# slothfulxtx/Texture-GS

Hardware: AMD Instinct MI355X
Metric: fwd+bwd views/sec @800x800, 300k Gaussians + 1024^2 texture; HBM GB/s vs roofline (higher is better)
Workload: dtype f32; 1 GPU; c3: N=300000 Gaussians, cubemap 6x1024x1024x3 f32, 800x800, fwd+bwd, sh_degree 3; parallelism=views sharded dp1, view_pipeline=3 HIP streams, order=accumulate, forwards begun one view per stream ahead, grad_allreduce=none (1 GPU)

## Files before the change

### texture-gs_amd/build.py

```python
import os
import subprocess
import sys

HERE = os.path.dirname(os.path.abspath(__file__))
ROOT = os.path.dirname(HERE)
CSRC = os.path.join(HERE, "csrc")
OBJ = os.path.join(HERE, "build")
LIB = os.path.join(HERE, os.environ.get("TEXGS_LIB_NAME", "libtexgs.so"))
OBJ = os.path.join(HERE, os.environ.get("TEXGS_OBJ_DIR", "build"))
HIPCC = os.environ.get("HIPCC", "/opt/rocm/bin/hipcc")

COMMON = ["--offload-arch=gfx950", "-O3", "-std=c++17", "-fPIC", "-I" + os.path.join(ROOT, "include"),
          "-I" + CSRC, "-Wall"]
UNITS = {
    "preprocess.hip": ["-ffp-contract=off"],
    "binning.hip": [],
    "render.hip": ["-munsafe-fp-atomics", "-ffp-contract=fast", "-fno-slp-vectorize"],
    "loss.hip": [],
    "selftest.hip": [],
    "uvnet.hip": [],
    "uvmap.hip": ["-munsafe-fp-atomics"],
    "points.hip": ["-ffp-contract=off"],
    "cubetex.hip": ["-munsafe-fp-atomics"],
    "density.hip": ["-ffp-contract=off"],
    "abi.hip": [],
}
HEADERS = [os.path.join(CSRC, "common.h"), os.path.join(CSRC, "wave_ops.h"), os.path.join(CSRC, "render_bwd_body.h"),
           os.path.join(ROOT, "include", "texgs.h")]


def build_id():
    import hashlib
    h = hashlib.sha256()
    files = sorted(os.path.join(CSRC, f) for f in os.listdir(CSRC) if f.endswith((".hip", ".h"))) + [os.path.join(ROOT, "include", "texgs.h")]
    for f in files:
        h.update(os.path.basename(f).encode())
        h.update(open(f, "rb").read())
    h.update(repr((COMMON[:4], sorted(UNITS.items()), os.environ.get("TEXGS_EXTRA_FLAGS", ""))).encode())
    return h.hexdigest()[:16]


def _newer(src_list, target):
    if not os.path.exists(target):
        return True
    t = os.path.getmtime(target)
    return any(os.path.getmtime(s) > t for s in src_list)


def build(force=False, verbose=False):
    os.makedirs(OBJ, exist_ok=True)
    objs = []
    bid = build_id()
    idfile = os.path.join(OBJ, "build_id.txt")
    stale_id = not os.path.exists(idfile) or open(idfile).read().strip() != bid
    for src, flags in UNITS.items():
        sp = os.path.join(CSRC, src)
        op = os.path.join(OBJ, src.replace(".hip", ".o"))
        objs.append(op)
        if src == "abi.hip":
            flags = flags + ['-DTEXGS_BUILD_ID="%s"' % bid]
# ... 18 lines not shown
```

### texture-gs_amd/csrc/abi.hip

```cpp
#include "common.h"
#include <stdio.h>
#include <string.h>
#include <stdlib.h>

#include <mutex>
#include <vector>

namespace {

thread_local char g_err[512] = "";

struct EvRec { int kid; hipEvent_t a, b; };
std::mutex g_prof_mu;
bool g_prof_on = false;
uint32_t g_prof_mask = 0xFFFFFFFFu;
std::vector<EvRec> g_prof_log;
std::vector<hipEvent_t> g_prof_free;

hipEvent_t prof_event() {
    if (!g_prof_free.empty()) { hipEvent_t e = g_prof_free.back(); g_prof_free.pop_back(); return e; }
    hipEvent_t e; (void)hipEventCreate(&e); return e;
}

struct ProfScope {
// ... 98 lines not shown
    const size_t nw = texgs_num_rendered_words(num_gaussians);
    if (host_words < nw) return fail_msg("host buffer too small (texgs_num_rendered_words)");
    hipStream_t s = (hipStream_t)stream;
    hipError_t e = hipMemcpyAsync(host_pinned, bin_block_sums_ptr(geom, num_gaussians), nw * sizeof(uint32_t), hipMemcpyDeviceToHost, s);
    if (e != hipSuccess) return fail("num_rendered readback", e);
    if (sort_first) {
        TexGSFrame f0; memset(&f0, 0, sizeof(f0)); f0.num_gaussians = num_gaussians;
        if (int r = depth_sort_scan(&f0, const_cast<TexGSGeom*>(geom), s)) return r;
    }
    return 0;
}
int texgs_num_rendered_reduce(const uint32_t* host_pinned, int32_t num_gaussians, uint32_t* host_out, uint64_t* fingerprint_out) {
    if (!host_pinned || !host_out) return fail_msg("NULL argument");
    *host_out = 0;
    if (fingerprint_out) *fingerprint_out = 0;
    if (num_gaussians <= 0) return 0;
    const size_t nblk = ((size_t)num_gaussians + TG_BLOCK - 1) / TG_BLOCK;
    unsigned long long total = 0ull;
    uint32_t fa = 0u, fb = 0u;
    for (size_t k = 0; k < nblk; ++k) { total += host_pinned[k]; fa += host_pinned[nblk + k]; fb += host_pinned[2 * nblk + k]; }
    if (total > 0xFFFFFFFFull) return fail_msg("num_rendered exceeds 2^32 - 1 instances");
    *host_out = (uint32_t)total;
    if (fingerprint_out) *fingerprint_out = ((uint64_t)fb << 32) | (uint64_t)fa;
    return 0;
}

int texgs_depth_sort_scan(TexGSGeom* geom, int32_t num_gaussians, void* stream) {
    if (!geom) return fail_msg("NULL argument");
    TexGSFrame f0; memset(&f0, 0, sizeof(f0)); f0.num_gaussians = num_gaussians;
    return depth_sort_scan(&f0, geom, (hipStream_t)stream);
}

static int render_forward_impl(const TexGSFrame* frame, const TexGSInputs* in, const TexGSGeom* geom,
                               const TexGSBinning* bin, TexGSImage* img, void* stream, bool counters_zeroed) {
    if (int r = validate_frame(frame)) return r;
    if (!in || !geom || !bin || !img) return fail_msg("NULL argument");
    hipStream_t s = (hipStream_t)stream;
    const CamConst c = make_cam(frame);
    if (img->tex_bin_count && in->texture && !counters_zeroed) {
        hipError_t e = hipMemsetAsync(img->tex_bin_count, 0, sizeof(uint32_t) * 2 * tex_bin_count(c.R), s);
        if (e != hipSuccess) return fail("tex_bin_count memset", e);
    }
    { ProfScope p(TEXGS_K_RENDER_FWD, s); launch_render_fwd(c, frame, in, geom, bin, img, s); }
    return check(frame, s, "render_fwd");
}

int texgs_render_forward(const TexGSFrame* frame, const TexGSInputs* in, const TexGSGeom* geom,
                         const TexGSBinning* bin, TexGSImage* img, void* stream) {
    return render_forward_impl(frame, in, geom, bin, img, stream, false);
}

int texgs_bin_sort_render_forward(const TexGSFrame* frame, const TexGSInputs* in, const TexGSGeom* geom,
                                  TexGSBinning* bin, TexGSImage* img, void* stream) {
    if (int r = validate_frame(frame)) return r;
    if (!in || !geom || !bin || !img) return fail_msg("NULL argument");
    hipStream_t s = (hipStream_t)stream;
    const CamConst c = make_cam(frame);
    if (bin->num_rendered > 0) {
        if (bin->sort_temp_bytes < sort_temp_bytes(bin->num_rendered, (uint32_t)(c.tiles_x * c.tiles_y))) return fail_msg("sort_temp too small");
        { ProfScope p(TEXGS_K_DUPLICATE, s); launch_duplicate(c, geom, bin, s); }
        if (int r = check(frame, s, "duplicate_with_keys")) return r;
        { ProfScope p(TEXGS_K_SORT, s);
          if (int r = launch_sort(c, geom, bin, s)) return fail("tile sort", (hipError_t)r); }
        if (int r = check(frame, s, "tile sort")) return r;
    }
    { ProfScope p(TEXGS_K_RANGES, s);
      launch_ranges(c, bin, img->tex_bin_count, img->tex_bin_count ? 2 * (int)tex_bin_count(c.R) : 0, s); }
    if (int r = check(frame, s, "tile_ranges")) return r;
    return render_forward_impl(frame, in, geom, bin, img, stream, true);
}

int texgs_backward_render(const TexGSFrame* frame, const TexGSInputs* in, const TexGSGeom* geom,
                          const TexGSBinning* bin, const TexGSImage* img, TexGSGrads* grads, void* stream) {
    if (int r = validate_frame(frame)) return r;
    if (!in || !geom || !bin || !img || !grads) return fail_msg("NULL argument");
    if (!(grads->want & TEXGS_WANT_ALL)) return fail_msg("TexGSGrads.want is empty: ask for TEXGS_WANT_TEXTURE and / or TEXGS_WANT_GAUSSIANS");
    if ((grads->want & TEXGS_WANT_GAUSSIANS) && !grads->acc) return fail_msg("acc must be allocated (zero-filled) when Gaussian gradients are wanted");
    if ((grads->want & TEXGS_WANT_TEXTURE) && in->texture && !grads->dL_dtexture) return fail_msg("dL_dtexture must be allocated (zero-filled) when the texture gradient is wanted");
    if (!img->survivors || !img->surv_qmask || !img->surv_count)
        return fail_msg("the forward of this call left no survivor lists (TexGSImage.survivors / surv_qmask / surv_count were NULL): "
                        "run the forward with them to be able to run its backward");
    hipStream_t s = (hipStream_t)stream;
    const CamConst c = make_cam(frame);
    if (bin->num_rendered > 0) {
        { ProfScope p(TEXGS_K_RENDER_BWD, s); launch_render_bwd(c, frame, in, geom, bin, img, grads, s); }
        if (int r = check(frame, s, "render_bwd")) return r;
        if (tex_bins_enabled(c, in, img, grads)) {
            { ProfScope p(TEXGS_K_TEXGRAD_REDUCE, s); launch_texgrad_reduce(c, img, grads, s); }
            if (int r = check(frame, s, "texgrad_reduce")) return r;
        }
    }
    return 0;
}

int texgs_backward_preprocess(const TexGSFrame* frame, const TexGSInputs* in, const TexGSGeom* geom, TexGSGrads* grads,
                              void* stream) {
    if (int r = validate_frame(frame)) return r;
    if (!in || !geom || !grads) return fail_msg("NULL argument");
    if (!(grads->want & TEXGS_WANT_GAUSSIANS)) return 0;
    if (!grads->acc) return fail_msg("acc must be allocated");
    if (in->cov3D_precomp && !grads->dL_dcov3D) return fail_msg("dL_dcov3D is required with cov3D_precomp");
    hipStream_t s = (hipStream_t)stream;
// ... 321 lines not shown
```

### texture-gs_amd/csrc/common.h

```cpp
#pragma once
#include <hip/hip_runtime.h>
#include <stdint.h>
#include "texgs.h"

#define TG_NEAR_Z        0.2f
#define TG_LOWPASS       0.3f
#define TG_FRUSTUM_CLAMP 1.3f
#define TG_ALPHA_MAX     0.99f
#define TG_ALPHA_MIN     (1.0f / 255.0f)
#define TG_T_EPS         1e-4f
#define TG_PLANE_EPS     5e-2f
#define TG_DEN_MIN       0.2f
#define TG_MA_MIN        1e-20f
#define TG_SH_C0         0.28209479177387814f

enum {
    R_XY = 0, R_CONIC = 2, R_OP = 5, R_G2 = 6, R_GM = 8, R_PHI = 14, R_VD = 17, R_DEPTH = 20, R_N = 21
};
enum {
    M_P = 0, M_DEN = 6, M_DN = 9, M_PHI = 18, M_VD = 21, M_DEPTH = 24, M_N = 25
};

#define TG_BLOCK 256

struct CamConst {
    int W, H, tiles_x, tiles_y;
    float fx, fy, tanfovx, tanfovy;
    float scale_modifier;
    int sh_degree, sh_coeffs, R, N;
};

static inline CamConst make_cam(const TexGSFrame* f) {
    CamConst c;
    c.W = f->image_width; c.H = f->image_height;
    c.tiles_x = (c.W + TEXGS_TILE - 1) / TEXGS_TILE;
    c.tiles_y = (c.H + TEXGS_TILE - 1) / TEXGS_TILE;
    c.tanfovx = f->tanfovx; c.tanfovy = f->tanfovy;
    c.fx = (float)c.W / (2.0f * f->tanfovx);
    c.fy = (float)c.H / (2.0f * f->tanfovy);
    c.scale_modifier = f->scale_modifier;
    c.sh_degree = f->sh_degree; c.sh_coeffs = f->sh_coeffs; c.R = f->tex_res; c.N = f->num_gaussians;
    return c;
}

void launch_preprocess_fwd(const CamConst& c, const TexGSFrame* f, const TexGSInputs* in, TexGSGeom* g, hipStream_t s);
void launch_preprocess_bwd(const CamConst& c, const TexGSFrame* f, const TexGSInputs* in, const TexGSGeom* g,
                           TexGSGrads* gr, hipStream_t s);
void launch_mark_visible(const TexGSFrame* f, const float* means3D, uint8_t* visible, hipStream_t s);
int  launch_depth_sort_scan(const TexGSGeom* g, int N, hipStream_t s);
uint32_t* bin_block_sums_ptr(const TexGSGeom* g, int N);
uint32_t* bin_header_ptr(const TexGSGeom* g, int N, int* words);
size_t scan_temp_bytes(int N);
size_t sort_temp_bytes(uint32_t D, uint32_t T);
void launch_duplicate(const CamConst& c, const TexGSGeom* g, TexGSBinning* b, hipStream_t s);
int  launch_sort(const CamConst& c, const TexGSGeom* g, TexGSBinning* b, hipStream_t s);
void launch_ranges(const CamConst& c, TexGSBinning* b, uint32_t* zero_words, int num_zero_words, hipStream_t s);
void launch_render_fwd(const CamConst& c, const TexGSFrame* f, const TexGSInputs* in, const TexGSGeom* g,
                       const TexGSBinning* b, TexGSImage* img, hipStream_t s);
size_t tex_bin_count(int R);
bool tex_bins_enabled(const CamConst& c, const TexGSInputs* in, const TexGSImage* img, const TexGSGrads* gr);
void launch_texgrad_reduce(const CamConst& c, const TexGSImage* img, TexGSGrads* gr, hipStream_t s);
void launch_render_bwd(const CamConst& c, const TexGSFrame* f, const TexGSInputs* in, const TexGSGeom* g,
                       const TexGSBinning* b, const TexGSImage* img, TexGSGrads* gr, hipStream_t s);
int launch_rgb_alpha_loss(const float* image, const float* gt_image, const float* alpha, const float* gt_alpha, int H,
                          int W, float lambda_dssim, float lambda_alpha, float* scratch, float* sums, float* d_image,
                          float* d_alpha, hipStream_t s);
void launch_selftest_waveops(const float* seed128, float* out576, hipStream_t s);
int launch_geom_losses(const float* norm, const float* gt_norm, const float* gt_image, const float* mask, const float* depth,
                       const float* gt_depth, int H, int W, float lambda_norm, float lambda_smooth, float gamma,
                       float lambda_depth, float* sums, float* d_norm, float* d_depth, hipStream_t s);
int launch_norm_from_depth(const float* depth, const float* viewmatrix, float tanfovx, float tanfovy, int H, int W, float threshold,
                           float* out_norm, float* out_mask, hipStream_t s);
size_t uv_packed_bytes(int precision);
int launch_uv_pack(const TexGSUVNet* net, int precision, void* packed, hipStream_t s);
int launch_uv_taylor_packed(const TexGSUVNet* net, int precision, const void* packed, const float* xyz, int N, float* uvs, float* grad_uvs,
                            hipStream_t s);
size_t uv_backward_temp_bytes(int N);
int launch_uv_backward(const TexGSUVNet* net, const float* xyz, const float* g, int N, const TexGSUVNetGrad* out, void* temp, int mixed,
                       hipStream_t s);
int hashgrid_levels(const TexGSHashGrid* g, float* scale, uint32_t* res, uint32_t* size, uint32_t* offset, uint32_t* n_params);
int launch_hashgrid_forward(const TexGSHashGrid* g, const float* params, const float* x, int N, float* enc, hipStream_t s);
size_t hashgrid_backward_temp_bytes(const TexGSHashGrid* g, int N);
int launch_hashgrid_backward(const TexGSHashGrid* g, const float* params, const float* x, const float* d_enc, int N, float* d_params,
                             float* d_x, void* temp, hipStream_t s);
size_t chamfer_nn_temp_bytes(int P);
int launch_chamfer_nn(const float* a, int P, const float* b, int Q, float* d2, int32_t* idx, void* temp, hipStream_t s);
size_t sort_pairs32_temp_bytes(uint32_t n);
int launch_sort_pairs32(const uint32_t* keys_in, uint32_t n, int key_bits, uint32_t* keys_out, uint32_t* vals_out, void* temp, hipStream_t s);
size_t knn3_temp_bytes(int n);
int launch_knn3_mean_dist2(const float* xyz, int n, float* mean_d2, void* temp, hipStream_t s);
// ... 12 lines not shown
```

### texture-gs_amd/csrc/render.hip

```cpp
#include "common.h"
#include "wave_ops.h"

namespace {

typedef unsigned long long ull;

struct __attribute__((packed, aligned(4))) Texel3 { float x, y, z; };
__device__ __forceinline__ Texel3 load_texel(const float* __restrict__ tex, uint32_t boff) {
    return *reinterpret_cast<const Texel3*>(reinterpret_cast<const char*>(tex) + boff);
}

typedef uint32_t tg_u4 __attribute__((ext_vector_type(4)));
template <class T> __device__ __forceinline__ T nt_load(const T* p) {
    return __builtin_nontemporal_load(p);
}
template <class T> __device__ __forceinline__ void nt_store(T* p, T v) {
    __builtin_nontemporal_store(v, p);
}
__device__ __forceinline__ uint2 nt_load2(const uint2* p) {
    const unsigned long long v = nt_load(reinterpret_cast<const unsigned long long*>(p));
    return make_uint2((uint32_t)v, (uint32_t)(v >> 32));
}
__device__ __forceinline__ void nt_store2(uint2* p, uint2 v) {
    nt_store(reinterpret_cast<unsigned long long*>(p), (unsigned long long)v.x | ((unsigned long long)v.y << 32));
}

struct CubeTap {
    uint32_t o00, dox, doy;
    int   x0, y0;
    float fx, fy;
    float sc, tc, h, rma, sm, su, sv;
    int   axis, face;
};

// ... 105 lines not shown
#define KEY_OX(K)  ((int)(((K) >> 14) & 7u))
#define KEY_OY(K)  ((int)(((K) >> 17) & 7u))

__device__ __forceinline__ void lane_pixel(int lane, int& ox, int& oy) {
    ox = (((lane >> 4) & 1) << 2) | (lane & 3);
    oy = (((lane >> 5) & 1) << 2) | ((lane >> 2) & 3);
}

__device__ __forceinline__ void load_chunk(const PixArgs& a, Planes& P, int lane, bool live, uint32_t id, uint32_t pos,
                                           float4& T0, float4& T1) {
    const float4 z = make_float4(0.f, 0.f, 0.f, 0.f);
    float4 S0 = z, S1 = z, S2 = z, S3 = z, S4 = z;
    T0 = z; T1 = make_float4(0.f, 0.f, -1.f, 1.f);
    if (live) {
        const float4* __restrict__ tp = a.rec_test + 2 * (size_t)id;
        const float4* __restrict__ sp = a.rec_shade + (TEXGS_REC_SHADE_FLOATS / 4) * (size_t)id;
        T0 = tp[0]; T1 = tp[1]; S0 = sp[0]; S1 = sp[1]; S2 = sp[2]; S3 = sp[3]; S4 = sp[4];
    }
    P.A[lane] = T0;
    { float* pb = reinterpret_cast<float*>(&P.B[lane]); pb[0] = T1.x; pb[1] = T1.y; pb[2] = __uint_as_float(pos); }
    P.C[lane] = make_float4(S3.z, S3.w, S4.x, S4.y);
    P.D[lane] = S0; P.E[lane] = S1; P.F[lane] = S2;
    P.G[lane] = make_float2(S3.x, S3.y);
}
__device__ __forceinline__ void init_dummy(Planes& P, int lane) {
    if (lane == 0) {
        const float4 z = make_float4(0.f, 0.f, 0.f, 0.f);
        P.A[TG_DUMMY] = z; P.B[TG_DUMMY] = make_float4(0.f, 0.f, __uint_as_float(0xFFFFFFFFu), 0.f); P.C[TG_DUMMY] = z;
        P.D[TG_DUMMY] = z; P.E[TG_DUMMY] = z; P.F[TG_DUMMY] = z; P.G[TG_DUMMY] = make_float2(0.f, 0.f);
    }
}

#define FQ_CAP 128
struct __attribute__((aligned(16))) FwdLds {
    Planes p;
    uint2 q[FQ_CAP];
    ull col[64 * 3];
    uint32_t ring[TG_RING];
    uint8_t list[4][64];
    uint32_t ccnt[TG_RESV / 2];
};

template <bool TAPS>
__global__ void __launch_bounds__(64, 4)
k_render_fwd(PixArgs a, float* __restrict__ out_color, float* __restrict__ out_depth, float* __restrict__ out_norm,
             float* __restrict__ out_alpha, float* __restrict__ final_T, uint32_t* __restrict__ n_contrib,
             uint32_t* __restrict__ bin_count) {
    __shared__ FwdLds L;
    const int lane = (int)threadIdx.x;
    int tile, wave;
    if (!wave_block(a, tile, wave)) return;
    const int tile_x = tile % a.tiles_x, tile_y = tile / a.tiles_x;
    const int wave_px = tile_x * TEXGS_TILE + ((wave & 1) << 3), wave_py = tile_y * TEXGS_TILE + ((wave >> 1) << 3);
    int ox, oy;
    lane_pixel(lane, ox, oy);
    const int px = wave_px + ox, py = wave_py + oy;
    const bool inside = (px < a.W) && (py < a.H);
    const float pxf = (float)px, pyf = (float)py;
    const float wpx = (float)wave_px, wpy = (float)wave_py;
    const uint2 range = a.ranges[tile];
    const int todo = (int)(range.y - range.x);
    const float* __restrict__ tex = a.texture;
    const uint32_t keybase = ((uint32_t)lane << 8) | ((uint32_t)ox << 14) | ((uint32_t)oy << 17);
    const uint8_t* mylist = L.list[lane >> 4];
    const int nbins_row = (a.R + 31) >> 5;

    L.col[lane * 3 + 0] = 0ull; L.col[lane * 3 + 1] = 0ull; L.col[lane * 3 + 2] = 0ull;
    resv_bin(L.p, lane) = TG_RESV_EMPTY;
    if (lane < TG_RESV / 2) L.ccnt[lane] = 0u;
    init_dummy(L.p, lane);
    __builtin_amdgcn_wave_barrier();

    bool done = !inside;
    ull done_mask = TG_BALLOT(!inside);
    float T = 1.0f;
    float Dp = 0.f, N0 = 0.f, N1 = 0.f, N2 = 0.f, Al = 0.f;
    uint32_t last = 0;
    int qhead = 0, qtail = 0;

    int pn = 0;
    int p_pl = 0;
    float p_w = 0.f, p_fx = 0.f, p_fy = 0.f, p_vd0 = 0.f, p_vd1 = 0.f, p_vd2 = 0.f;
    Texel3 p00 = {0.f, 0.f, 0.f}, p01 = p00, p10 = p00, p11 = p00;
    auto finish = [&]() {
        if (lane < pn) {
            float t0 = 0.f, t1 = 0.f, t2 = 0.f;
            if constexpr (TAPS) {
                const float w00 = (1.f - p_fx) * (1.f - p_fy), w01 = p_fx * (1.f - p_fy);
                const float w10 = (1.f - p_fx) * p_fy,         w11 = p_fx * p_fy;
                t0 = w00 * p00.x + w01 * p01.x + w10 * p10.x + w11 * p11.x;
                t1 = w00 * p00.y + w01 * p01.y + w10 * p10.y + w11 * p11.y;
                t2 = w00 * p00.z + w01 * p01.z + w10 * p10.z + w11 * p11.z;
            }
            ull* cp = L.col + p_pl * 3;
            atomicAdd(cp + 0, (ull)(fminf(p_w * fmaxf(0.f, TG_SH_C0 * t0 + p_vd0 + 0.5f), 2.0e9f) * 4294967296.0f));
            atomicAdd(cp + 1, (ull)(fminf(p_w * fmaxf(0.f, TG_SH_C0 * t1 + p_vd1 + 0.5f), 2.0e9f) * 4294967296.0f));
            atomicAdd(cp + 2, (ull)(fminf(p_w * fmaxf(0.f, TG_SH_C0 * t2 + p_vd2 + 0.5f), 2.0e9f) * 4294967296.0f));
        }
        pn = 0;
    };
    auto drain = [&](int n_) {
        finish();
        uint2 e_ = make_uint2(0u, 0u);
        if (lane < n_) e_ = L.q[(qhead + lane) & (FQ_CAP - 1)];
        const int jj_ = KEY_J(e_.y);
        const float4 f_ = L.p.F[jj_];
        const float2 g2 = L.p.G[jj_];
        const float4 a4_ = L.p.A[jj_];
        const float2 b2_ = *reinterpret_cast<const float2*>(&L.p.B[jj_]);
        const float ipx_ = (float)(wave_px + KEY_OX(e_.y)), ipy_ = (float)(wave_py + KEY_OY(e_.y));
        const float araw_ = gauss_alpha_raw(b2_.y, gauss_power(a4_.z, a4_.w, b2_.x, a4_.x - ipx_, a4_.y - ipy_));
        const float T_ = __uint_as_float(e_.x);
        const float w_ = fminf(TG_ALPHA_MAX, araw_) * T_;
        if constexpr (TAPS) {
            const float2 xy = make_float2(a4_.x, a4_.y);
            const float4 d_ = L.p.D[jj_], e4 = L.p.E[jj_];
            const float dpx = ipx_ - xy.x, dpy = ipy_ - xy.y;
            const float den = 1.0f + d_.x * dpx + d_.y * dpy;
            const float inv = (den >= TG_DEN_MIN) ? __builtin_amdgcn_rcpf(den) : 0.0f;
            const float u0 = f_.x + (d_.z * dpx + d_.w * dpy) * inv;
            const float u1 = f_.y + (e4.x * dpx + e4.y * dpy) * inv;
            const float u2 = f_.z + (e4.z * dpx + e4.w * dpy) * inv;
            const CubeTap ct = cube_address(u0, u1, u2, a.R);
            p00 = load_texel(tex, ct.o00); p01 = load_texel(tex, ct.o00 + ct.dox);
            p10 = load_texel(tex, ct.o00 + ct.doy); p11 = load_texel(tex, ct.o00 + ct.doy + ct.dox);
            p_fx = ct.fx; p_fy = ct.fy;
            if (bin_count != nullptr) {
                const bool binned = (lane < n_) && tap_binned(ct);
                const uint32_t bin = tap_bin(ct, nbins_row);
                const int home = tap_home(ct);
                const bool hit = binned && resv_bin(L.p, home) == bin;
                if (hit) atomicAdd(&L.ccnt[home >> 1], 1u << ((home & 1) << 4));
                ull pend = TG_BALLOT(binned) & ~TG_BALLOT(hit);
                while (pend != 0ull) {
                    const int l0 = __ffsll((long long)pend) - 1;
                    const uint32_t b0 = (uint32_t)__builtin_amdgcn_readlane((int)bin, l0);
                    const int h0 = __builtin_amdgcn_readlane(home, l0);
                    const ull m = pend & TG_BALLOT(bin == b0);
                    const uint32_t e0 = resv_bin(L.p, h0);
                    if (lane == l0) {
                        const uint32_t n = (uint32_t)__popcll(m);
                        if (e0 == TG_RESV_EMPTY) { resv_bin(L.p, h0) = b0; atomicAdd(&L.ccnt[h0 >> 1], n << ((h0 & 1) << 4)); }
                        else atomicAdd(bin_count + 6 * nbins_row * nbins_row + b0, n);
                    }
                    __builtin_amdgcn_wave_barrier();
                    pend &= ~m;
                }
            }
        }
        p_w = w_; p_pl = KEY_PL(e_.y); p_vd0 = f_.w; p_vd1 = g2.x; p_vd2 = g2.y;
        pn = n_;
    };

    const size_t sbase = 4 * (size_t)range.x + (size_t)wave * (size_t)todo;
    int nsurv = 0;
    int r = 0, nq = 0, qh = 0;
    const float4 zt0 = make_float4(0.f, 0.f, 0.f, 0.f), zt1 = make_float4(0.f, 0.f, -1.f, 1.f);
    float4 nt0 = zt0, nt1 = zt1;
    if (lane < todo) {
        const float4* __restrict__ tp = a.rec_test + 2 * (size_t)a.point_list[range.x + lane];
        nt0 = tp[0]; nt1 = tp[1];
    }
    uint32_t nid = (64 + lane < todo) ? a.point_list[range.x + 64 + lane] : 0u;
    bool all_done = (~done_mask == 0ull);
    while (!all_done) {
        while (nq < 64 && r < todo) {
            const int idx = r + lane;
            const float4 t0 = nt0, t1 = nt1;
            r += 64;
            nt0 = zt0; nt1 = zt1;
            if (r + lane < todo) {
                const float4* __restrict__ tp = a.rec_test + 2 * (size_t)nid;
                nt0 = tp[0]; nt1 = tp[1];
            }
            nid = (r + 64 + lane < todo) ? a.point_list[range.x + r + 64 + lane] : 0u;
            const bool reach = block_reachable(t0.x, t0.y, t0.z, t0.w, t1.x, t1.w, t1.z, wpx, wpy, 7.0f);
            const ull m = TG_BALLOT(reach);
            if (reach) L.ring[(qh + nq + mbcnt64(m)) & (TG_RING - 1)] = (uint32_t)idx;
            nq += __popcll(m);
        }
        if (nq == 0) break;
        const int take = min(64, nq);
        __builtin_amdgcn_wave_barrier();
        uint32_t pos = 0xFFFFFFFFu, id = 0u;
        if (lane < take) {
            pos = L.ring[(qh + lane) & (TG_RING - 1)];
            id = a.point_list[range.x + pos];
        }
        qh = (qh + take) & (TG_RING - 1); nq -= take;
        float4 T0, T1;
        load_chunk(a, L.p, lane, lane < take, id, pos, T0, T1);
        reinterpret_cast<uint32_t*>(&L.list[0][0])[lane] = 0x40404040u;
        __builtin_amdgcn_wave_barrier();
        int len[4];
        uint32_t qbits = 0u;
#pragma unroll
        for (int q = 0; q < 4; ++q) {
            const bool rowdone = ((done_mask >> (16 * q)) & 0xFFFFull) == 0xFFFFull;
            const bool geo = (lane < take) &&
                block_reachable(T0.x, T0.y, T0.z, T0.w, T1.x, T1.w, T1.z, wpx + (float)((q & 1) << 2), wpy + (float)((q >> 1) << 2), 3.0f);
            qbits |= geo ? (1u << q) : 0u;
            const bool rq = geo && !rowdone;
            const ull m = TG_BALLOT(rq);
            len[q] = __popcll(m);
            if (rq) L.list[q][mbcnt64(m)] = (uint8_t)lane;
        }
        if (a.surv != nullptr) {
            if (lane < take) { nt_store2(a.surv + sbase + nsurv + lane, make_uint2(id, pos)); nt_store(a.surv_qm + sbase + nsurv + lane, (uint16_t)qbits); }
            nsurv += take;
        }
        __builtin_amdgcn_wave_barrier();
        int tmax = max(max(len[0], len[1]), max(len[2], len[3]));
        auto test_one = [&](const float4& A, const float4& B, const float4& Cc, const int j) -> bool {
                const float power = gauss_power(A.z, A.w, B.x, A.x - pxf, A.y - pyf);
                const float alpha = fminf(TG_ALPHA_MAX, gauss_alpha_raw(B.y, power));
                const ull m_ok = TG_BALLOT(power <= 0.0f) & ~done_mask & TG_BALLOT(alpha >= TG_ALPHA_MIN);
                if (m_ok == 0ull) return false;
                bool ok = (!done) && (power <= 0.0f) && (alpha >= TG_ALPHA_MIN);
                const float Tn = T * (1.0f - alpha);
                const ull m_kill = m_ok & TG_BALLOT(Tn < TG_T_EPS);
                if (ok && Tn < TG_T_EPS) { done = true; ok = false; }
                done_mask |= m_kill;
                const ull bal = m_ok & ~m_kill;
                if (bal != 0ull) {
                    if (ok) {
                        const float w = alpha * T;
                        Dp += w * Cc.x; N0 += w * Cc.y; N1 += w * Cc.z; N2 += w * Cc.w; Al += w;
                        L.q[(qtail + mbcnt64(bal)) & (FQ_CAP - 1)] = make_uint2(__float_as_uint(T), keybase | (uint32_t)j);
                        T = Tn;
                        last = __float_as_uint(B.z) + 1u;
                    }
                    qtail += __popcll(bal);
                    if (qtail - qhead >= 64) {
                        __builtin_amdgcn_wave_barrier();
                        drain(64);
                        qhead += 64;
                    }
                }
                if (m_kill != 0ull) {
                    if (~done_mask == 0ull) { all_done = true; return true; }
// ... 5 lines not shown
                }
            return false;
        };
        int jx = mylist[0], jy = mylist[1];
        float4 xA = L.p.A[jx], xB = L.p.B[jx], xC = L.p.C[jx];
        float4 yA = xA, yB = xB, yC = xC;
        for (int t = 0; t < tmax; t += 2) {
            yA = L.p.A[jy]; yB = L.p.B[jy]; yC = L.p.C[jy];
            const int j0 = jx;
            jx = mylist[min(t + 2, 63)];
            if (test_one(xA, xB, xC, j0)) break;
            if (t + 1 >= tmax) break;
            xA = L.p.A[jx]; xB = L.p.B[jx]; xC = L.p.C[jx];
            const int j1 = jy;
            jy = mylist[min(t + 3, 63)];
            if (test_one(yA, yB, yC, j1)) break;
        }
        if (qtail - qhead > 0) {
            __builtin_amdgcn_wave_barrier();
            drain(qtail - qhead);
            qhead = qtail;
        }
        __builtin_amdgcn_wave_barrier();
    }
    finish();
    __builtin_amdgcn_wave_barrier();
    if (TAPS && bin_count != nullptr) {
        const uint32_t b = resv_bin(L.p, lane), n = (L.ccnt[lane >> 1] >> ((lane & 1) << 4)) & 0xFFFFu;
        uint32_t off = 0u;
        if (b != TG_RESV_EMPTY) off = atomicAdd(bin_count + b, n);
        uint32_t* __restrict__ rv = a.resv + (size_t)(4 * tile + wave) * (3 * TG_RESV);
        nt_store(rv + lane, b); nt_store(rv + TG_RESV + lane, off); nt_store(rv + 2 * TG_RESV + lane, n);
    }
    if (a.surv_cnt != nullptr && lane == 0) a.surv_cnt[4 * tile + wave] = (uint32_t)nsurv;
    if (inside) {
        const int HW = a.W * a.H, pix = py * a.W + px;
        const double q = 1.0 / 4294967296.0;
        nt_store(out_color + pix, (float)((double)L.col[lane * 3 + 0] * q) + T * a.bg[0]);
        nt_store(out_color + HW + pix, (float)((double)L.col[lane * 3 + 1] * q) + T * a.bg[1]);
        nt_store(out_color + 2 * HW + pix, (float)((double)L.col[lane * 3 + 2] * q) + T * a.bg[2]);
        nt_store(out_depth + pix, Dp);
        nt_store(out_norm + pix, N0); nt_store(out_norm + HW + pix, N1); nt_store(out_norm + 2 * HW + pix, N2);
        nt_store(out_alpha + pix, Al);
        nt_store(final_T + pix, T);
        nt_store(n_contrib + pix, last);
    }
}

#define BWD_MAX_IT 16
struct TexBinArgs {
    uint32_t* rec;
    uint32_t* cursor;
    const uint32_t* base;
    const uint32_t* order;
    uint32_t* stats;
    uint32_t  cap;
    int       nb;
};

__device__ __forceinline__ void scatter_direct(float* __restrict__ dtex, uint32_t o00, uint32_t dox, uint32_t doy, float fx, float fy,
                                               float x0, float x1, float x2) {
    const float w00 = (1.f - fx) * (1.f - fy), w01 = fx * (1.f - fy), w10 = (1.f - fx) * fy, w11 = fx * fy;
    float* p00 = dtex + (o00 >> 2);
    float* p01 = dtex + ((o00 + dox) >> 2);
    float* p10 = dtex + ((o00 + doy) >> 2);
    float* p11 = dtex + ((o00 + doy + dox) >> 2);
    unsafeAtomicAdd(p00, w00 * x0); unsafeAtomicAdd(p00 + 1, w00 * x1); unsafeAtomicAdd(p00 + 2, w00 * x2);
    unsafeAtomicAdd(p01, w01 * x0); unsafeAtomicAdd(p01 + 1, w01 * x1); unsafeAtomicAdd(p01 + 2, w01 * x2);
    unsafeAtomicAdd(p10, w10 * x0); unsafeAtomicAdd(p10 + 1, w10 * x1); unsafeAtomicAdd(p10 + 2, w10 * x2);
    unsafeAtomicAdd(p11, w11 * x0); unsafeAtomicAdd(p11 + 1, w11 * x1); unsafeAtomicAdd(p11 + 2, w11 * x2);
}

struct __attribute__((aligned(16))) Rec4 { uint32_t a, b, c, d; };
__device__ __forceinline__ void rec_store(uint32_t* __restrict__ base, uint32_t slot, const Rec4 r) {
    tg_u4 v; v.x = r.a; v.y = r.b; v.z = r.c; v.w = r.d;
    __builtin_nontemporal_store(v, reinterpret_cast<tg_u4*>(base) + slot);
}
__device__ __forceinline__ Rec4 rec_load(const Rec4* __restrict__ p) {
    const tg_u4 v = __builtin_nontemporal_load(reinterpret_cast<const tg_u4*>(p));
// ... 190 lines not shown
    a.rec_test = reinterpret_cast<const float4*>(g->rec_test);
    a.rec_shade = reinterpret_cast<const float4*>(g->rec_shade);
    a.texture = in->texture;
    a.bg = f->bg;
    const bool hand = img->survivors != nullptr && img->surv_qmask != nullptr && img->surv_count != nullptr;
    a.surv = hand ? reinterpret_cast<uint2*>(img->survivors) : nullptr;
    a.surv_qm = hand ? img->surv_qmask : nullptr;
    a.surv_cnt = hand ? img->surv_count : nullptr;
    a.resv = img->tex_bin_resv;
    return a;
}

inline TexBinArgs make_bins(const CamConst& c, const TexGSImage* img, const TexGSGrads* gr) {
    TexBinArgs tb;
    tb.nb = (c.R + 31) >> 5;
    const bool on = (gr->want & TEXGS_WANT_TEXTURE) && img->tex_bin_count != nullptr && img->tex_bin_resv != nullptr && gr->tex_bins != nullptr &&
                    gr->tex_bin_cursor != nullptr && gr->tex_bin_base != nullptr && gr->tex_rec_cap > 0;
    tb.rec = on ? reinterpret_cast<uint32_t*>(gr->tex_bins) : nullptr;
    tb.cursor = on ? gr->tex_bin_cursor : nullptr;
    tb.base = on ? gr->tex_bin_base : nullptr;
    tb.order = on ? gr->tex_bin_base + tex_bin_count(c.R) + 1 : nullptr;
    tb.stats = on ? gr->tex_bin_cursor + tex_bin_count(c.R) : nullptr;
    tb.cap = on ? gr->tex_rec_cap : 0u;
    return tb;
}

}

size_t tex_bin_count(int R) {
    const size_t nb = (size_t)((R + 31) >> 5);
    return 6 * nb * nb;
}

void launch_render_fwd(const CamConst& c, const TexGSFrame* f, const TexGSInputs* in, const TexGSGeom* g,
                       const TexGSBinning* b, TexGSImage* img, hipStream_t s) {
    const PixArgs a = make_pix(c, f, in, g, b, img);
    if (in->texture)
        hipLaunchKernelGGL(k_render_fwd<true>, dim3(blend_grid(a.num_tiles)), dim3(64), 0, s, a, img->out_color, img->out_depth,
                           img->out_norm, img->out_alpha, img->final_T, img->n_contrib, img->tex_bin_resv ? img->tex_bin_count : (uint32_t*)nullptr);
    else
        hipLaunchKernelGGL(k_render_fwd<false>, dim3(blend_grid(a.num_tiles)), dim3(64), 0, s, a, img->out_color, img->out_depth,
                           img->out_norm, img->out_alpha, img->final_T, img->n_contrib, (uint32_t*)nullptr);
}

void launch_render_bwd(const CamConst& c, const TexGSFrame* f, const TexGSInputs* in, const TexGSGeom* g,
                       const TexGSBinning* b, const TexGSImage* img, TexGSGrads* gr, hipStream_t s) {
    const PixArgs a = make_pix(c, f, in, g, b, img);
    const TexBinArgs tb = make_bins(c, img, gr);
    const bool taps = in->texture != nullptr;
    const bool tex = taps && (gr->want & TEXGS_WANT_TEXTURE) && gr->dL_dtexture != nullptr;
    const bool geo = (gr->want & TEXGS_WANT_GAUSSIANS) != 0;
    if (!tex && !geo) return;
    if (tex && tb.rec)
        hipLaunchKernelGGL(k_bin_offsets, dim3(1), dim3(1024), 0, s, (int)tex_bin_count(c.R), (const uint32_t*)img->tex_bin_count,
                           gr->tex_bin_base, gr->tex_bin_cursor, gr->tex_bin_base + tex_bin_count(c.R) + 1, tb.stats);
    const dim3 grid(blend_grid(a.num_tiles)), blk(64);
#define K7_LAUNCH(NS, TEX, GEO, UVG, TAPS) hipLaunchKernelGGL((NS::k_render_bwd<TEX, GEO, UVG, TAPS>), grid, blk, 0, s, a, tb, img->final_T, \
        img->n_contrib, gr->dL_dcolor, gr->dL_ddepth, gr->dL_dnorm, gr->dL_dalpha, gr->acc, gr->dL_dtexture)
    if (!taps)            K7_LAUNCH(k7_occ, false, true, false, false);
    else if (tex && geo)  K7_LAUNCH(k7_occ, true, true, true, true);
    else if (tex)         K7_LAUNCH(k7_lds, true, false, false, true);
    else                  K7_LAUNCH(k7_occ, false, true, true, true);
#undef K7_LAUNCH
}

bool tex_bins_enabled(const CamConst& c, const TexGSInputs* in, const TexGSImage* img, const TexGSGrads* gr) {
    return in->texture != nullptr && gr->dL_dtexture != nullptr && make_bins(c, img, gr).rec != nullptr;
}

void launch_texgrad_reduce(const CamConst& c, const TexGSImage* img, TexGSGrads* gr, hipStream_t s) {
    const TexBinArgs tb = make_bins(c, img, gr);
    if (!tb.rec) return;
    hipLaunchKernelGGL(k_texgrad_reduce, dim3((unsigned)tex_bin_count(c.R)), dim3(TB_THREADS), 0, s, c.R, tb, gr->dL_dtexture);
}

// ... 6 lines not shown
```

Baseline: 1016 views/s.

## Add per-tile block-cull prepass feeding precomputed survivor lists to forward render

Result: no change. 1021 views/s, median of 3 (+0.5%).

```diff
diff --git a/texture-gs_amd/build.py b/texture-gs_amd/build.py
--- a/texture-gs_amd/build.py
+++ b/texture-gs_amd/build.py
@@ -25,7 +25,7 @@
     "density.hip": ["-ffp-contract=off"],
     "abi.hip": [],
 }
-HEADERS = [os.path.join(CSRC, "common.h"), os.path.join(CSRC, "wave_ops.h"), os.path.join(CSRC, "render_bwd_body.h"),
+HEADERS = [os.path.join(CSRC, "common.h"), os.path.join(CSRC, "wave_ops.h"), os.path.join(CSRC, "render_bwd_body.h"), os.path.join(CSRC, "q32.h"),
            os.path.join(ROOT, "include", "texgs.h")]
 
 
diff --git a/texture-gs_amd/csrc/abi.hip b/texture-gs_amd/csrc/abi.hip
--- a/texture-gs_amd/csrc/abi.hip
+++ b/texture-gs_amd/csrc/abi.hip
@@ -154,7 +154,7 @@
 }
 
 static int render_forward_impl(const TexGSFrame* frame, const TexGSInputs* in, const TexGSGeom* geom,
-                               const TexGSBinning* bin, TexGSImage* img, void* stream, bool counters_zeroed) {
+                               const TexGSBinning* bin, TexGSImage* img, void* stream, bool counters_zeroed, bool preculled) {
     if (int r = validate_frame(frame)) return r;
     if (!in || !geom || !bin || !img) return fail_msg("NULL argument");
     hipStream_t s = (hipStream_t)stream;
@@ -163,13 +163,13 @@
         hipError_t e = hipMemsetAsync(img->tex_bin_count, 0, sizeof(uint32_t) * 2 * tex_bin_count(c.R), s);
         if (e != hipSuccess) return fail("tex_bin_count memset", e);
     }
-    { ProfScope p(TEXGS_K_RENDER_FWD, s); launch_render_fwd(c, frame, in, geom, bin, img, s); }
+    { ProfScope p(TEXGS_K_RENDER_FWD, s); launch_render_fwd(c, frame, in, geom, bin, img, preculled, s); }
     return check(frame, s, "render_fwd");
 }
 
 int texgs_render_forward(const TexGSFrame* frame, const TexGSInputs* in, const TexGSGeom* geom,
                          const TexGSBinning* bin, TexGSImage* img, void* stream) {
-    return render_forward_impl(frame, in, geom, bin, img, stream, false);
+    return render_forward_impl(frame, in, geom, bin, img, stream, false, false);
 }
 
 int texgs_bin_sort_render_forward(const TexGSFrame* frame, const TexGSInputs* in, const TexGSGeom* geom,
@@ -186,10 +186,12 @@
           if (int r = launch_sort(c, geom, bin, s)) return fail("tile sort", (hipError_t)r); }
         if (int r = check(frame, s, "tile sort")) return r;
     }
+    const bool preculled = block_cull_applies(img);
     { ProfScope p(TEXGS_K_RANGES, s);
-      launch_ranges(c, bin, img->tex_bin_count, img->tex_bin_count ? 2 * (int)tex_bin_count(c.R) : 0, s); }
-    if (int r = check(frame, s, "tile_ranges")) return r;
-    return render_forward_impl(frame, in, geom, bin, img, stream, true);
+      launch_ranges(c, bin, img->tex_bin_count, img->tex_bin_count ? 2 * (int)tex_bin_count(c.R) : 0, s);
+      if (preculled) launch_block_cull(c, frame, in, geom, bin, img, s); }
+    if (int r = check(frame, s, "tile_ranges / block_cull")) return r;
+    return render_forward_impl(frame, in, geom, bin, img, stream, true, preculled);
 }
 
 int texgs_backward_render(const TexGSFrame* frame, const TexGSInputs* in, const TexGSGeom* geom,
diff --git a/texture-gs_amd/csrc/common.h b/texture-gs_amd/csrc/common.h
--- a/texture-gs_amd/csrc/common.h
+++ b/texture-gs_amd/csrc/common.h
@@ -56,6 +56,9 @@
 int  launch_sort(const CamConst& c, const TexGSGeom* g, TexGSBinning* b, hipStream_t s);
 void launch_ranges(const CamConst& c, TexGSBinning* b, uint32_t* zero_words, int num_zero_words, hipStream_t s);
 void launch_render_fwd(const CamConst& c, const TexGSFrame* f, const TexGSInputs* in, const TexGSGeom* g,
+                       const TexGSBinning* b, TexGSImage* img, bool preculled, hipStream_t s);
+bool block_cull_applies(const TexGSImage* img);
+void launch_block_cull(const CamConst& c, const TexGSFrame* f, const TexGSInputs* in, const TexGSGeom* g,
                        const TexGSBinning* b, TexGSImage* img, hipStream_t s);
 size_t tex_bin_count(int R);
 bool tex_bins_enabled(const CamConst& c, const TexGSInputs* in, const TexGSImage* img, const TexGSGrads* gr);
diff --git a/texture-gs_amd/csrc/q32.h b/texture-gs_amd/csrc/q32.h
--- /dev/null
+++ b/texture-gs_amd/csrc/q32.h
@@ -0,0 +1,14 @@
+#pragma once
+#include <stdint.h>
+
+#if defined(__HIPCC__)
+#define TG_Q32_FN __host__ __device__ __forceinline__
+#else
+#define TG_Q32_FN static inline
+#endif
+
+TG_Q32_FN uint64_t q32_from_float(float x) {
+    const uint32_t hi = (uint32_t)x;
+    const uint32_t lo = (uint32_t)((x - (float)hi) * 4294967296.0f);
+    return ((uint64_t)hi << 32) | (uint64_t)lo;
+}
diff --git a/texture-gs_amd/csrc/render.hip b/texture-gs_amd/csrc/render.hip
--- a/texture-gs_amd/csrc/render.hip
+++ b/texture-gs_amd/csrc/render.hip
@@ -1,5 +1,7 @@
 #include "common.h"
 #include "wave_ops.h"
+#include "q32.h"
+#include <stdlib.h>
 
 namespace {
 
@@ -171,7 +173,8 @@
 }
 
 #define FQ_CAP 128
-struct __attribute__((aligned(16))) FwdLds {
+template <bool PRECULLED> struct FwdLds;
+template <> struct __attribute__((aligned(16))) FwdLds<false> {
     Planes p;
     uint2 q[FQ_CAP];
     ull col[64 * 3];
@@ -179,13 +182,20 @@
     uint8_t list[4][64];
     uint32_t ccnt[TG_RESV / 2];
 };
-
-template <bool TAPS>
+template <> struct __attribute__((aligned(16))) FwdLds<true> {
+    Planes p;
+    uint2 q[FQ_CAP];
+    ull col[64 * 3];
+    uint8_t list[4][64];
+    uint32_t ccnt[TG_RESV / 2];
+};
+
+template <bool TAPS, bool PRECULLED>
 __global__ void __launch_bounds__(64, 4)
 k_render_fwd(PixArgs a, float* __restrict__ out_color, float* __restrict__ out_depth, float* __restrict__ out_norm,
              float* __restrict__ out_alpha, float* __restrict__ final_T, uint32_t* __restrict__ n_contrib,
              uint32_t* __restrict__ bin_count) {
-    __shared__ FwdLds L;
+    __shared__ FwdLds<PRECULLED> L;
     const int lane = (int)threadIdx.x;
     int tile, wave;
     if (!wave_block(a, tile, wave)) return;
@@ -197,6 +207,7 @@
     const bool inside = (px < a.W) && (py < a.H);
     const float pxf = (float)px, pyf = (float)py;
     const float wpx = (float)wave_px, wpy = (float)wave_py;
+    (void)wpx; (void)wpy;
     const uint2 range = a.ranges[tile];
     const int todo = (int)(range.y - range.x);
     const float* __restrict__ tex = a.texture;
@@ -232,9 +243,9 @@
                 t2 = w00 * p00.z + w01 * p01.z + w10 * p10.z + w11 * p11.z;
             }
             ull* cp = L.col + p_pl * 3;
-            atomicAdd(cp + 0, (ull)(fminf(p_w * fmaxf(0.f, TG_SH_C0 * t0 + p_vd0 + 0.5f), 2.0e9f) * 4294967296.0f));
-            atomicAdd(cp + 1, (ull)(fminf(p_w * fmaxf(0.f, TG_SH_C0 * t1 + p_vd1 + 0.5f), 2.0e9f) * 4294967296.0f));
-            atomicAdd(cp + 2, (ull)(fminf(p_w * fmaxf(0.f, TG_SH_C0 * t2 + p_vd2 + 0.5f), 2.0e9f) * 4294967296.0f));
+            atomicAdd(cp + 0, (ull)q32_from_float(fminf(p_w * fmaxf(0.f, TG_SH_C0 * t0 + p_vd0 + 0.5f), 2.0e9f)));
+            atomicAdd(cp + 1, (ull)q32_from_float(fminf(p_w * fmaxf(0.f, TG_SH_C0 * t1 + p_vd1 + 0.5f), 2.0e9f)));
+            atomicAdd(cp + 2, (ull)q32_from_float(fminf(p_w * fmaxf(0.f, TG_SH_C0 * t2 + p_vd2 + 0.5f), 2.0e9f)));
         }
         pn = 0;
     };
@@ -294,39 +305,60 @@
     const size_t sbase = 4 * (size_t)range.x + (size_t)wave * (size_t)todo;
     int nsurv = 0;
     int r = 0, nq = 0, qh = 0;
+    (void)r; (void)nq; (void)qh;
     const float4 zt0 = make_float4(0.f, 0.f, 0.f, 0.f), zt1 = make_float4(0.f, 0.f, -1.f, 1.f);
     float4 nt0 = zt0, nt1 = zt1;
-    if (lane < todo) {
-        const float4* __restrict__ tp = a.rec_test + 2 * (size_t)a.point_list[range.x + lane];
-        nt0 = tp[0]; nt1 = tp[1];
-    }
-    uint32_t nid = (64 + lane < todo) ? a.point_list[range.x + 64 + lane] : 0u;
+    uint32_t nid = 0u;
+    int ns = 0, c0 = 0;
+    uint2 nsv = make_uint2(0u, 0xFFFFFFFFu);
+    uint32_t nqm = 0u;
+    if constexpr (PRECULLED) {
+        ns = min((int)a.surv_cnt[4 * tile + wave], todo);
+        if (lane < ns) { nsv = nt_load2(a.surv + sbase + lane); nqm = nt_load(a.surv_qm + sbase + lane); }
+    } else {
+        if (lane < todo) {
+            const float4* __restrict__ tp = a.rec_test + 2 * (size_t)a.point_list[range.x + lane];
+            nt0 = tp[0]; nt1 = tp[1];
+        }
+        nid = (64 + lane < todo) ? a.point_list[range.x + 64 + lane] : 0u;
+    }
     bool all_done = (~done_mask == 0ull);
     while (!all_done) {
-        while (nq < 64 && r < todo) {
-            const int idx = r + lane;
-            const float4 t0 = nt0, t1 = nt1;
-            r += 64;
-            nt0 = zt0; nt1 = zt1;
-            if (r + lane < todo) {
-                const float4* __restrict__ tp = a.rec_test + 2 * (size_t)nid;
-                nt0 = tp[0]; nt1 = tp[1];
+        int take;
+        uint32_t pos = 0xFFFFFFFFu, id = 0u, qm = 0u;
+        (void)qm;
+        if constexpr (PRECULLED) {
+            if (c0 >= ns) break;
+            take = min(64, ns - c0);
+            id = nsv.x; pos = nsv.y; qm = nqm;
+            c0 += 64;
+            nsv = make_uint2(0u, 0xFFFFFFFFu); nqm = 0u;
+            if (c0 + lane < ns) { nsv = nt_load2(a.surv + sbase + c0 + lane); nqm = nt_load(a.surv_qm + sbase + c0 + lane); }
+        } else {
+            while (nq < 64 && r < todo) {
+                const int idx = r + lane;
+                const float4 t0 = nt0, t1 = nt1;
+                r += 64;
+                nt0 = zt0; nt1 = zt1;
+                if (r + lane < todo) {
+                    const float4* __restrict__ tp = a.rec_test + 2 * (size_t)nid;
+                    nt0 = tp[0]; nt1 = tp[1];
+                }
+                nid = (r + 64 + lane < todo) ? a.point_list[range.x + r + 64 + lane] : 0u;
+                const bool reach = block_reachable(t0.x, t0.y, t0.z, t0.w, t1.x, t1.w, t1.z, wpx, wpy, 7.0f);
+                const ull m = TG_BALLOT(reach);
+                if (reach) L.ring[(qh + nq + mbcnt64(m)) & (TG_RING - 1)] = (uint32_t)idx;
+                nq += __popcll(m);
             }
-            nid = (r + 64 + lane < todo) ? a.point_list[range.x + r + 64 + lane] : 0u;
-            const bool reach = block_reachable(t0.x, t0.y, t0.z, t0.w, t1.x, t1.w, t1.z, wpx, wpy, 7.0f);
-            const ull m = TG_BALLOT(reach);
-            if (reach) L.ring[(qh + nq + mbcnt64(m)) & (TG_RING - 1)] = (uint32_t)idx;
-            nq += __popcll(m);
-        }
-        if (nq == 0) break;
-        const int take = min(64, nq);
-        __builtin_amdgcn_wave_barrier();
-        uint32_t pos = 0xFFFFFFFFu, id = 0u;
-        if (lane < take) {
-            pos = L.ring[(qh + lane) & (TG_RING - 1)];
-            id = a.point_list[range.x + pos];
-        }
-        qh = (qh + take) & (TG_RING - 1); nq -= take;
+            if (nq == 0) break;
+            take = min(64, nq);
+            __builtin_amdgcn_wave_barrier();
+            if (lane < take) {
+                pos = L.ring[(qh + lane) & (TG_RING - 1)];
+                id = a.point_list[range.x + pos];
+            }
+            qh = (qh + take) & (TG_RING - 1); nq -= take;
+        }
         float4 T0, T1;
         load_chunk(a, L.p, lane, lane < take, id, pos, T0, T1);
         reinterpret_cast<uint32_t*>(&L.list[0][0])[lane] = 0x40404040u;
@@ -336,7 +368,9 @@
 #pragma unroll
         for (int q = 0; q < 4; ++q) {
             const bool rowdone = ((done_mask >> (16 * q)) & 0xFFFFull) == 0xFFFFull;
-            const bool geo = (lane < take) &&
+            bool geo;
+            if constexpr (PRECULLED) geo = ((qm >> q) & 1u) != 0u;
+            else geo = (lane < take) &&
                 block_reachable(T0.x, T0.y, T0.z, T0.w, T1.x, T1.w, T1.z, wpx + (float)((q & 1) << 2), wpy + (float)((q >> 1) << 2), 3.0f);
             qbits |= geo ? (1u << q) : 0u;
             const bool rq = geo && !rowdone;
@@ -344,7 +378,7 @@
             len[q] = __popcll(m);
             if (rq) L.list[q][mbcnt64(m)] = (uint8_t)lane;
         }
-        if (a.surv != nullptr) {
+        if (!PRECULLED && a.surv != nullptr) {
             if (lane < take) { nt_store2(a.surv + sbase + nsurv + lane, make_uint2(id, pos)); nt_store(a.surv_qm + sbase + nsurv + lane, (uint16_t)qbits); }
             nsurv += take;
         }
@@ -416,7 +450,7 @@
         uint32_t* __restrict__ rv = a.resv + (size_t)(4 * tile + wave) * (3 * TG_RESV);
         nt_store(rv + lane, b); nt_store(rv + TG_RESV + lane, off); nt_store(rv + 2 * TG_RESV + lane, n);
     }
-    if (a.surv_cnt != nullptr && lane == 0) a.surv_cnt[4 * tile + wave] = (uint32_t)nsurv;
+    if (!PRECULLED && a.surv_cnt != nullptr && lane == 0) a.surv_cnt[4 * tile + wave] = (uint32_t)nsurv;
     if (inside) {
         const int HW = a.W * a.H, pix = py * a.W + px;
         const double q = 1.0 / 4294967296.0;
@@ -429,6 +463,98 @@
         nt_store(final_T + pix, T);
         nt_store(n_contrib + pix, last);
     }
+}
+
+#define BC_THREADS 256
+struct __attribute__((aligned(16))) CullLds {
+    float4 t0[BC_THREADS], t1[BC_THREADS];
+    uint8_t src[4][BC_THREADS];
+    uint32_t cnt[BC_THREADS / 64][4];
+};
+__global__ void __launch_bounds__(BC_THREADS)
+k_block_cull(PixArgs a) {
+    __shared__ CullLds L;
+    const int tid = (int)threadIdx.x, lane = tid & 63, wv = tid >> 6;
+    const int tile = (int)a.tile_order[blockIdx.x];
+    const uint2 range = a.ranges[tile];
+    const int todo = (int)(range.y - range.x);
+    const int tile_px = (tile % a.tiles_x) * TEXGS_TILE, tile_py = (tile / a.tiles_x) * TEXGS_TILE;
+    float bx[4], by[4];
+    bool bin[4];
+#pragma unroll
+    for (int b = 0; b < 4; ++b) {
+        const int x = tile_px + ((b & 1) << 3), y = tile_py + ((b >> 1) << 3);
+        bx[b] = (float)x; by[b] = (float)y;
+        bin[b] = (x < a.W) && (y < a.H);
+    }
+    const size_t sb0 = 4 * (size_t)range.x;
+    uint32_t run[4] = {0u, 0u, 0u, 0u};
+    const float4 zt0 = make_float4(0.f, 0.f, 0.f, 0.f), zt1 = make_float4(0.f, 0.f, -1.f, 1.f);
+    float4 nt0 = zt0, nt1 = zt1;
+    uint32_t cid = 0u;
+    if (tid < todo) {
+        cid = a.point_list[range.x + tid];
+        const float4* __restrict__ tp = a.rec_test + 2 * (size_t)cid;
+        nt0 = tp[0]; nt1 = tp[1];
+    }
+    uint32_t nid = (BC_THREADS + tid < todo) ? a.point_list[range.x + BC_THREADS + tid] : 0u;
+    for (int r0 = 0; r0 < todo; r0 += BC_THREADS) {
+        const int idx = r0 + tid;
+        const float4 t0 = nt0, t1 = nt1;
+        const uint32_t id = cid;
+        cid = nid; nt0 = zt0; nt1 = zt1;
+        if (idx + BC_THREADS < todo) {
+            const float4* __restrict__ tp = a.rec_test + 2 * (size_t)nid;
+            nt0 = tp[0]; nt1 = tp[1];
+        }
+        nid = (idx + 2 * BC_THREADS < todo) ? a.point_list[range.x + idx + 2 * BC_THREADS] : 0u;
+        L.t0[tid] = t0; L.t1[tid] = t1;
+        bool reach[4];
+        ull m[4];
+#pragma unroll
+        for (int b = 0; b < 4; ++b) {
+            reach[b] = bin[b] && block_reachable(t0.x, t0.y, t0.z, t0.w, t1.x, t1.w, t1.z, bx[b], by[b], 7.0f);
+            m[b] = TG_BALLOT(reach[b]);
+        }
+        if (lane == 0) {
+#pragma unroll
+            for (int b = 0; b < 4; ++b) L.cnt[wv][b] = (uint32_t)__popcll(m[b]);
+        }
+        __syncthreads();
+        uint32_t tot[4];
+#pragma unroll
+        for (int b = 0; b < 4; ++b) {
+            uint32_t before = 0u, all = 0u;
+#pragma unroll
+            for (int w = 0; w < BC_THREADS / 64; ++w) { const uint32_t c = L.cnt[w][b]; all += c; before += (w < wv) ? c : 0u; }
+            tot[b] = all;
+            if (reach[b]) {
+                const uint32_t k = before + (uint32_t)mbcnt64(m[b]);
+                a.surv[sb0 + (size_t)b * (size_t)todo + run[b] + k] = make_uint2(id, (uint32_t)idx);
+                L.src[b][k] = (uint8_t)tid;
+            }
+        }
+        __syncthreads();
+        const uint32_t p1 = tot[0], p2 = p1 + tot[1], p3 = p2 + tot[2], p4 = p3 + tot[3];
+        for (uint32_t j = (uint32_t)tid; j < p4; j += BC_THREADS) {
+            const int b = (int)(j >= p1) + (int)(j >= p2) + (int)(j >= p3);
+            const uint32_t k = j - (b == 0 ? 0u : b == 1 ? p1 : b == 2 ? p2 : p3);
+            const uint32_t rb = b == 0 ? run[0] : b == 1 ? run[1] : b == 2 ? run[2] : run[3];
+            const float x0 = (b & 1) ? bx[1] : bx[0], y0 = (b & 2) ? by[2] : by[0];
+            const int sl = (int)L.src[b][k];
+            const float4 T0 = L.t0[sl], T1 = L.t1[sl];
+            uint32_t qbits = 0u;
+#pragma unroll
+            for (int q = 0; q < 4; ++q)
+                qbits |= block_reachable(T0.x, T0.y, T0.z, T0.w, T1.x, T1.w, T1.z, x0 + (float)((q & 1) << 2), y0 + (float)((q >> 1) << 2), 3.0f)
+                             ? (1u << q) : 0u;
+            a.surv_qm[sb0 + (size_t)b * (size_t)todo + rb + k] = (uint16_t)qbits;
+        }
+#pragma unroll
+        for (int b = 0; b < 4; ++b) run[b] += tot[b];
+        __syncthreads();
+    }
+    if (tid < 4) a.surv_cnt[4 * tile + tid] = tid == 0 ? run[0] : tid == 1 ? run[1] : tid == 2 ? run[2] : run[3];
 }
 
 #define BWD_MAX_IT 16
@@ -685,15 +811,29 @@
     return 6 * nb * nb;
 }
 
-void launch_render_fwd(const CamConst& c, const TexGSFrame* f, const TexGSInputs* in, const TexGSGeom* g,
+bool block_cull_applies(const TexGSImage* img) {
+    if (!(img->survivors != nullptr && img->surv_qmask != nullptr && img->surv_count != nullptr)) return false;
+    const char* e = getenv("TEXGS_PRECULL");
+    return !(e != nullptr && e[0] == '0' && e[1] == '\0');
+}
+
+void launch_block_cull(const CamConst& c, const TexGSFrame* f, const TexGSInputs* in, const TexGSGeom* g,
                        const TexGSBinning* b, TexGSImage* img, hipStream_t s) {
     const PixArgs a = make_pix(c, f, in, g, b, img);
-    if (in->texture)
-        hipLaunchKernelGGL(k_render_fwd<true>, dim3(blend_grid(a.num_tiles)), dim3(64), 0, s, a, img->out_color, img->out_depth,
-                           img->out_norm, img->out_alpha, img->final_T, img->n_contrib, img->tex_bin_resv ? img->tex_bin_count : (uint32_t*)nullptr);
-    else
-        hipLaunchKernelGGL(k_render_fwd<false>, dim3(blend_grid(a.num_tiles)), dim3(64), 0, s, a, img->out_color, img->out_depth,
-                           img->out_norm, img->out_alpha, img->final_T, img->n_contrib, (uint32_t*)nullptr);
+    if (a.surv == nullptr || a.num_tiles <= 0) return;
+    hipLaunchKernelGGL(k_block_cull, dim3(a.num_tiles), dim3(BC_THREADS), 0, s, a);
+}
+
+void launch_render_fwd(const CamConst& c, const TexGSFrame* f, const TexGSInputs* in, const TexGSGeom* g,
+                       const TexGSBinning* b, TexGSImage* img, bool preculled, hipStream_t s) {
+    const PixArgs a = make_pix(c, f, in, g, b, img);
+    preculled = preculled && a.surv != nullptr;
+    uint32_t* const bins = (in->texture && img->tex_bin_resv) ? img->tex_bin_count : (uint32_t*)nullptr;
+#define K6_LAUNCH(TAPS, PRE) hipLaunchKernelGGL((k_render_fwd<TAPS, PRE>), dim3(blend_grid(a.num_tiles)), dim3(64), 0, s, a, img->out_color, \
+        img->out_depth, img->out_norm, img->out_alpha, img->final_T, img->n_contrib, bins)
+    if (in->texture) { if (preculled) K6_LAUNCH(true, true); else K6_LAUNCH(true, false); }
+    else             { if (preculled) K6_LAUNCH(false, true); else K6_LAUNCH(false, false); }
+#undef K6_LAUNCH
 }
 
 void launch_render_bwd(const CamConst& c, const TexGSFrame* f, const TexGSInputs* in, const TexGSGeom* g,
```
